# gaocegege/kubeflow-controller

Measured on AMD Instinct MI355X. Metric: images/sec (whole node) ResNet-50 TFJob at 1/2/4/8 workers on MI355X, higher is better.
Workload: dtype bf16; 1 GPU; model=ResNet-50 v1.5, global_batch=256, image=224, per_gpu_batch=256, parallelism=single, optimizer=SGD momentum 0.9 (fused HIP), fp32 master, hip_graph=False

## Files before the change

### csrc/kernels/batchnorm.hip

```cpp
#include <cstdlib>

#include "common.h"

namespace {

constexpr int NT = 256;
constexpr int kSlots = 64;

struct Geom {
  int tpr;
  int rpi;
  int gx;
  long chunk;
};

Geom geom(long M, int C, int max_blocks) {
  Geom g;
  int cv = C / 8;
  g.tpr = cv < NT ? cv : NT;
  g.rpi = NT / g.tpr;
  long want = (M + (long)g.rpi * 8 - 1) / ((long)g.rpi * 8);
  long gx = want < max_blocks ? want : max_blocks;
  if (gx < 1) gx = 1;
  long chunk = (M + gx - 1) / gx;
// ... 266 lines not shown
  {
    const Geom ga = apply_geom(M, C);
    grid = dim3(ga.gx);
    chunk = ga.chunk;
    tpr = ga.tpr;
    rpi = ga.rpi;
  }
  if (rss && relu && res && mb)
    hipLaunchKernelGGL((bn_apply<true, true, true, true>), grid, dim3(NT), 0, s, x, res, y, mb, scale, shift, M, C,
                       chunk, tpr, rpi, rss);
  else if (rss && relu && res)
    hipLaunchKernelGGL((bn_apply<true, true, false, true>), grid, dim3(NT), 0, s, x, res, y, mb, scale, shift, M, C,
                       chunk, tpr, rpi, rss);
  else if (rss && res)
    hipLaunchKernelGGL((bn_apply<false, true, false, true>), grid, dim3(NT), 0, s, x, res, y, mb, scale, shift, M, C,
                       chunk, tpr, rpi, rss);
  else if (relu && res && mb)
    hipLaunchKernelGGL((bn_apply<true, true, true>), grid, dim3(NT), 0, s, x, res, y, mb, scale, shift, M, C, chunk,
                       tpr, rpi);
  else if (relu && res)
    hipLaunchKernelGGL((bn_apply<true, true, false>), grid, dim3(NT), 0, s, x, res, y, mb, scale, shift, M, C, chunk,
                       tpr, rpi);
  else if (relu)
    hipLaunchKernelGGL((bn_apply<true, false, false>), grid, dim3(NT), 0, s, x, res, y, mb, scale, shift, M, C, chunk,
                       tpr, rpi);
  else if (res)
    hipLaunchKernelGGL((bn_apply<false, true, false>), grid, dim3(NT), 0, s, x, res, y, mb, scale, shift, M, C, chunk,
                       tpr, rpi);
  else
    hipLaunchKernelGGL((bn_apply<false, false, false>), grid, dim3(NT), 0, s, x, res, y, mb, scale, shift, M, C,
                       chunk, tpr, rpi);
}

template <int MASK>
__device__ __forceinline__ void masked_dy(const uint4 dv, const uint4 yv, const float xf[8], const float sc[8],
                                          const float sf[8], unsigned bits, float dz[8]) {
  unpack8(dv, dz);
  if (MASK == 3) {
#pragma unroll
    for (int j = 0; j < 8; j++) dz[j] = ((bits >> j) & 1u) ? dz[j] : 0.f;
  } else if (MASK == 1) {
    float yy[8];
    unpack8(yv, yy);
#pragma unroll
    for (int j = 0; j < 8; j++) dz[j] = yy[j] > 0.f ? dz[j] : 0.f;
  } else if (MASK == 2) {
#pragma unroll
    for (int j = 0; j < 8; j++) dz[j] = fmaf(xf[j], sc[j], sf[j]) > 0.f ? dz[j] : 0.f;
  }
}

template <int MASK>
__device__ __forceinline__ void load_ss(const float* __restrict__ ss, int C, int c0, float sc[8], float sf[8]) {
#pragma unroll
  for (int j = 0; j < 8; j++) {
    sc[j] = MASK == 2 ? ss[c0 + j] : 0.f;
    sf[j] = MASK == 2 ? ss[C + c0 + j] : 0.f;
  }
}

template <int MASK>
__global__ __launch_bounds__(NT) void bn_bwd_partial(const bf16_t* __restrict__ dy, const bf16_t* __restrict__ x,
                                                     const bf16_t* __restrict__ y, const uint8_t* __restrict__ mb,
                                                     const float* __restrict__ ss,
                                                     const float* __restrict__ mean, float* __restrict__ part, long M,
                                                     int C, long chunk, int tpr, int rpi) {
  __shared__ __attribute__((aligned(16))) float sh[kRedFloats];
  const int t = threadIdx.x;
  const int cg = t % tpr, r0 = t / tpr;
  const bool active = r0 < rpi;
  const int cv = C / 8;
  const long rb = (long)blockIdx.x * chunk;
  const long re = rb + chunk < M ? rb + chunk : M;
  for (int g0 = 0; g0 < cv; g0 += tpr) {
    const int c0 = (g0 + cg) * 8;
    float s1[8] = {0, 0, 0, 0, 0, 0, 0, 0}, s2[8] = {0, 0, 0, 0, 0, 0, 0, 0};
    if (active && g0 + cg < cv) {
      float mu[8], sc[8], sf[8];
#pragma unroll
      for (int j = 0; j < 8; j++) mu[j] = mean[c0 + j];
      load_ss<MASK>(ss, C, c0, sc, sf);
      long r = rb + r0;
      for (; r + rpi < re; r += 2L * rpi) {
// ... 442 lines not shown
```

### csrc/kernels/common.h

```cpp
#pragma once
#include <hip/hip_runtime.h>
#include <stdint.h>

#define KFA_API extern "C" __attribute__((visibility("default")))

typedef uint16_t bf16_t;
typedef __attribute__((ext_vector_type(8))) short short8;
typedef __attribute__((ext_vector_type(4))) float floatx4;
typedef __attribute__((ext_vector_type(16))) float floatx16;

__device__ __forceinline__ float bf2f(uint32_t b) { return __uint_as_float(b << 16); }

typedef __attribute__((ext_vector_type(2))) __bf16 kfa_bf16x2_t;
typedef __attribute__((ext_vector_type(2))) float kfa_floatx2_t;

__device__ __forceinline__ uint32_t pack2(float lo, float hi) {
  const kfa_floatx2_t f = {lo, hi};
  return __builtin_bit_cast(uint32_t, __builtin_convertvector(f, kfa_bf16x2_t));
}

__device__ __forceinline__ uint32_t f2bf(float f) { return pack2(f, 0.f) & 0xffffu; }

__device__ __forceinline__ void unpack8(const uint4 v, float f[8]) {
  f[0] = __uint_as_float(v.x << 16); f[1] = __uint_as_float(v.x & 0xffff0000u);
  f[2] = __uint_as_float(v.y << 16); f[3] = __uint_as_float(v.y & 0xffff0000u);
  f[4] = __uint_as_float(v.z << 16); f[5] = __uint_as_float(v.z & 0xffff0000u);
  f[6] = __uint_as_float(v.w << 16); f[7] = __uint_as_float(v.w & 0xffff0000u);
}

__device__ __forceinline__ uint4 pack8(const float f[8]) {
  return make_uint4(pack2(f[0], f[1]), pack2(f[2], f[3]), pack2(f[4], f[5]), pack2(f[6], f[7]));
}

__device__ __forceinline__ float wave_sum(float v) {
#pragma unroll
  for (int o = 32; o > 0; o >>= 1) v += __shfl_xor(v, o, 64);
  return v;
}

__device__ __forceinline__ float wave_max(float v) {
#pragma unroll
  for (int o = 32; o > 0; o >>= 1) v = fmaxf(v, __shfl_xor(v, o, 64));
  return v;
}

__device__ __forceinline__ float erf_as(float x, float& e) {
  const float a = fabsf(x);
  const float t = __builtin_amdgcn_rcpf(fmaf(0.3275911f, a, 1.f));
  e = __expf(-a * a);
  const float poly =
      t * fmaf(t, fmaf(t, fmaf(t, fmaf(t, 1.061405429f, -1.453152027f), 1.421413741f), -0.284496736f), 0.254829592f);
  return copysignf(1.f - poly * e, x);
}
__device__ __forceinline__ float gelu_f(float z) {
  float e;
  return 0.5f * z * (1.f + erf_as(z * 0.70710678118654752f, e));
}
__device__ __forceinline__ float gelu_grad(float z) {
  float e;
  const float cdf = 0.5f * (1.f + erf_as(z * 0.70710678118654752f, e));
  return fmaf(z * 0.39894228040143268f, e, cdf);
}

__device__ __forceinline__ uint32_t drop_hash(uint64_t seed, uint64_t i) {
// ... 24 lines not shown
```

### csrc/kernels/pool.hip

```cpp
#include <cstdlib>

#include "common.h"

namespace {

template <typename IT>
__global__ __launch_bounds__(256) void maxpool_fwd(const bf16_t* __restrict__ x, bf16_t* __restrict__ y,
                                                   uint8_t* __restrict__ idx, int N, int H, int W, int C, int Ho,
                                                   int Wo, int k, int s, int p) {
  const IT cv = C / 8;
  const IT total = (IT)N * Ho * Wo * cv;
  for (IT v = (IT)blockIdx.x * blockDim.x + threadIdx.x; v < total; v += (IT)gridDim.x * blockDim.x) {
    const int cg = (int)(v % cv);
    IT t = v / cv;
    const int ow = (int)(t % (IT)Wo);
    t /= (IT)Wo;
    const int oh = (int)(t % (IT)Ho);
    const int n = (int)(t / (IT)Ho);
    float best[8];
    int bi[8];
#pragma unroll
    for (int j = 0; j < 8; j++) { best[j] = -INFINITY; bi[j] = 0; }
    for (int kh = 0; kh < k; kh++) {
      const int ih = oh * s - p + kh;
// ... 212 lines not shown
  for (int a = 0; a < 2; a++)
#pragma unroll
    for (int b = 0; b < 2; b++) {
      const int oh = oh1 - a, ow = ow1 - b;
      const int kh = ih - (oh * 2 - p), kw = iw - (ow * 2 - p);
      const int w = a * 2 + b;
      ok[w] = oh >= 0 && oh < Ho && ow >= 0 && ow < Wo && kh < 3 && kw < 3;
      pos[w] = kh * 3 + kw;
      const long o = (((long)n * Ho + min(max(oh, 0), Ho - 1)) * Wo + min(max(ow, 0), Wo - 1)) * C + cg * 8;
      g[w] = *reinterpret_cast<const uint4*>(dy + o);
      pk[w] = *reinterpret_cast<const uint2*>(idx + o);
    }
  float acc[8] = {0, 0, 0, 0, 0, 0, 0, 0};
#pragma unroll
  for (int w = 0; w < 4; w++) {
    if (!ok[w]) continue;
    float f[8];
    unpack8(g[w], f);
    const uint32_t q[2] = {pk[w].x, pk[w].y};
#pragma unroll
    for (int j = 0; j < 8; j++)
      if ((int)((q[j >> 2] >> ((j & 3) * 8)) & 0xff) == pos[w]) acc[j] += f[j];
  }
  *reinterpret_cast<uint4*>(dx + (long)v * 8) = pack8(acc);
}

struct PoolBnStats {
  const bf16_t* x;
  const float* ss;
  const float* mean;
  float* slots;
};

template <bool STATS>
__global__ __launch_bounds__(256) void maxpool3s2_bwd4(const bf16_t* __restrict__ dy, const uint8_t* __restrict__ idx,
                                                       bf16_t* __restrict__ dx, int N, int H, int W, int C, int Ho,
                                                       int Wo, int p, int T, int U, PoolBnStats bs) {
  const unsigned cv = C / 8;
  const unsigned total = (unsigned)N * T * U * cv;
  const unsigned v = blockIdx.x * blockDim.x + threadIdx.x;
  if (!STATS && v >= total) return;
  const bool live = v < total;
  float s1[8] = {0, 0, 0, 0, 0, 0, 0, 0}, s2[8] = {0, 0, 0, 0, 0, 0, 0, 0};
  float mu[8], sc[8], sf[8];
  const int cg = (int)(v % cv);
  if (STATS)
#pragma unroll
    for (int j = 0; j < 8; j++) {
      mu[j] = bs.mean[cg * 8 + j];
      sc[j] = bs.ss[cg * 8 + j];
      sf[j] = bs.ss[C + cg * 8 + j];
    }
  unsigned q = v / cv;
  const int u = (int)(q % (unsigned)U);
  q /= (unsigned)U;
  const int t = (int)(q % (unsigned)T);
  const int n = live ? (int)(q / (unsigned)T) : 0;
  uint4 g[4];
  uint2 pk[4];
  bool ok[4];
#pragma unroll
  for (int b = 0; b < 2; b++)
#pragma unroll
    for (int e = 0; e < 2; e++) {
      const int oh = t - 1 + b, ow = u - 1 + e, w = b * 2 + e;
      ok[w] = live && oh >= 0 && oh < Ho && ow >= 0 && ow < Wo;
      const long o = (((long)n * Ho + min(max(oh, 0), Ho - 1)) * Wo + min(max(ow, 0), Wo - 1)) * C + cg * 8;
      g[w] = *reinterpret_cast<const uint4*>(dy + o);
      pk[w] = *reinterpret_cast<const uint2*>(idx + o);
    }
#pragma unroll
  for (int a = 0; a < 2; a++)
#pragma unroll
    for (int c = 0; c < 2; c++) {
      const int ih = 2 * t - p + a, iw = 2 * u - p + c;
      if (!live || ih < 0 || ih >= H || iw < 0 || iw >= W) continue;
      float acc[8] = {0, 0, 0, 0, 0, 0, 0, 0};
#pragma unroll
      for (int b = 0; b < 2; b++)
#pragma unroll
        for (int e = 0; e < 2; e++) {
          const int kh = a + 2 - 2 * b, kw = c + 2 - 2 * e;
          const int w = b * 2 + e;
          if (kh > 2 || kw > 2 || !ok[w]) continue;
          const int pos = kh * 3 + kw;
          float f[8];
          unpack8(g[w], f);
          const uint32_t qq[2] = {pk[w].x, pk[w].y};
#pragma unroll
          for (int j = 0; j < 8; j++)
            if ((int)((qq[j >> 2] >> ((j & 3) * 8)) & 0xff) == pos) acc[j] += f[j];
        }
      const long o = (((long)n * H + ih) * W + iw) * C + cg * 8;
      const uint4 packed = pack8(acc);
      *reinterpret_cast<uint4*>(dx + o) = packed;
      if (STATS) {
        float dz[8], xf[8];
        unpack8(packed, dz);
        unpack8(*reinterpret_cast<const uint4*>(bs.x + o), xf);
#pragma unroll
        for (int j = 0; j < 8; j++) {
          const float d = fmaf(xf[j], sc[j], sf[j]) > 0.f ? dz[j] : 0.f;
          s1[j] += d;
          s2[j] += d * (xf[j] - mu[j]);
        }
      }
    }
  if (STATS) {
#pragma unroll
    for (int o = 8; o < 64; o <<= 1)
#pragma unroll
      for (int j = 0; j < 8; j++) { s1[j] += __shfl_xor(s1[j], o, 64); s2[j] += __shfl_xor(s2[j], o, 64); }
    const int lane = threadIdx.x & 63, jj = lane >> 3;
    float a1 = s1[0], a2 = s2[0];
#pragma unroll
    for (int j = 1; j < 8; j++) {
      a1 = jj == j ? s1[j] : a1;
      a2 = jj == j ? s2[j] : a2;
    }
    const int ch = (lane & 7) * 8 + jj;
    float* slot = bs.slots + (long)(blockIdx.x % 64) * 2 * C;
    __hip_atomic_fetch_add(slot + ch, a1, __ATOMIC_RELAXED, __HIP_MEMORY_SCOPE_AGENT);
    __hip_atomic_fetch_add(slot + C + ch, a2, __ATOMIC_RELAXED, __HIP_MEMORY_SCOPE_AGENT);
  }
}

bool pool_bwd4() {
  static int v = -1;
  if (v < 0) {
    const char* e = getenv("KFA_POOL_BWD4");
    v = (e && e[0] == '0') ? 0 : 1;
  }
  return v == 1;
}

int grid_for(long work) {
  long b = (work + 255) / 256;
  return (int)(b < (1L << 20) ? (b < 1 ? 1 : b) : (1L << 20));
}

bool pool_pairs() {
  static int v = -1;
  if (v < 0) {
    const char* e = getenv("KFA_POOL_PAIRS");
    v = (e && e[0] == '0') ? 0 : 1;
  }
  return v == 1;
}

}

KFA_API int kfa_maxpool_fwd(const bf16_t* x, bf16_t* y, uint8_t* idx, int N, int H, int W, int C, int Ho, int Wo,
                            int k, int s, int p, hipStream_t st) {
  if (C % 8 || k > 15) return -1;
  const long work = (long)N * Ho * Wo * (C / 8);
  if (k == 3 && s == 2 && p <= 1 && work < (1L << 31) && (long)N * H * W * C < (1L << 40) && pool_pairs())
    hipLaunchKernelGGL(maxpool3s2_fwd2<false>, dim3((unsigned)(((long)N * Ho * ((Wo + 1) / 2) * (C / 8) + 255) / 256)),
// ... 12 lines not shown

KFA_API int kfa_maxpool_bwd(const bf16_t* dy, const uint8_t* idx, bf16_t* dx, int N, int H, int W, int C, int Ho,
                            int Wo, int k, int s, int p, hipStream_t st) {
  if (C % 8 || k > 15) return -1;
  const long work = (long)N * H * W * (C / 8);
  const int T = (H + p + 1) / 2, U = (W + p + 1) / 2;
  const long work4 = (long)N * T * U * (C / 8);
  if (k == 3 && s == 2 && p <= 1 && pool_bwd4() && work4 < (1L << 31))
    hipLaunchKernelGGL(maxpool3s2_bwd4<false>, dim3((unsigned)((work4 + 255) / 256)), dim3(256), 0, st, dy, idx, dx, N,
                       H, W, C, Ho, Wo, p, T, U, PoolBnStats{nullptr, nullptr, nullptr, nullptr});
  else if (k == 3 && s == 2 && p <= 1 && work < (1L << 31))
    hipLaunchKernelGGL(maxpool3s2_bwd, dim3((unsigned)((work + 255) / 256)), dim3(256), 0, st, dy, idx, dx, N, H, W, C,
                       Ho, Wo, p);
  else if (work < (1L << 31))
    hipLaunchKernelGGL(maxpool_bwd<unsigned>, dim3(grid_for(work)), dim3(256), 0, st, dy, idx, dx, N, H, W, C, Ho, Wo,
                       k, s, p);
  else
    hipLaunchKernelGGL(maxpool_bwd<long>, dim3(grid_for(work)), dim3(256), 0, st, dy, idx, dx, N, H, W, C, Ho, Wo, k,
                       s, p);
  return kfa_status();
}

KFA_API int kfa_maxpool_bwd_bnstats(const bf16_t* dy, const uint8_t* idx, bf16_t* dx, int N, int H, int W, int C,
                                    int Ho, int Wo, int p, const bf16_t* x, const float* ss, const float* mean,
                                    float* slots, hipStream_t st) {
  const int T = (H + p + 1) / 2, U = (W + p + 1) / 2;
  const long work4 = (long)N * T * U * (C / 8);
  if (C != 64 || p > 1 || work4 >= (1L << 31) || !x || !ss || !mean || !slots) return -1;
  hipLaunchKernelGGL(maxpool3s2_bwd4<true>, dim3((unsigned)((work4 + 255) / 256)), dim3(256), 0, st, dy, idx, dx, N, H,
                     W, C, Ho, Wo, p, T, U, PoolBnStats{x, ss, mean, slots});
  return kfa_status();
}

KFA_API int kfa_maxpool_fwd_bn(const bf16_t* x, bf16_t* y, uint8_t* idx, int N, int H, int W, int C, int Ho, int Wo,
                               int k, int s, int p, const float* ss, hipStream_t st) {
  const long work = (long)N * Ho * Wo * (C / 8);
  if (C % 8 || k != 3 || s != 2 || p > 1 || !ss || work >= (1L << 31) || (long)N * H * W * C >= (1L << 40)) return -1;
  if (pool_pairs()) {
    const long w2 = (long)N * Ho * ((Wo + 1) / 2) * (C / 8);
    hipLaunchKernelGGL(maxpool3s2_fwd2<true>, dim3((unsigned)((w2 + 255) / 256)), dim3(256), 0, st, x, y, idx, N, H,
                       W, C, Ho, Wo, p, ss);
  } else {
    hipLaunchKernelGGL(maxpool3s2_fwd<true>, dim3((unsigned)((work + 255) / 256)), dim3(256), 0, st, x, y, idx, N, H,
                       W, C, Ho, Wo, p, ss);
  }
  return kfa_status();
}

namespace {
__global__ __launch_bounds__(256) void gap_fwd_kernel(const bf16_t* __restrict__ x, bf16_t* __restrict__ y, int N, int HW,
                                                      int C) {
  const int cv = C / 8;
  const int t = blockIdx.x * blockDim.x + threadIdx.x;
  if (t >= N * cv) return;
  const int n = t / cv, c8 = t - n * cv;
  const bf16_t* p = x + (long)n * HW * C + c8 * 8;
  float s[8] = {0.f, 0.f, 0.f, 0.f, 0.f, 0.f, 0.f, 0.f};
  int i = 0;
  for (; i + 3 < HW; i += 4) {
    uint4 v[4];
#pragma unroll
    for (int u = 0; u < 4; u++) v[u] = *reinterpret_cast<const uint4*>(p + (long)(i + u) * C);
#pragma unroll
    for (int u = 0; u < 4; u++) {
      float f[8];
      unpack8(v[u], f);
// ... 48 lines not shown
```

### kubeflow_controller_amd/ops/batchnorm.py

```python
from __future__ import annotations

import os

import torch
import torch.nn as nn

from . import _lib
from ..parallel.flat import direct_grad_view, notify_grad_ready


MASK_FROM_X = os.environ.get("KFA_BN_MASK_FROM_X", "1") != "0"


def _as_rows(t: torch.Tensor) -> torch.Tensor:
    if t.dim() == 4:
        if not t.is_contiguous(memory_format=torch.channels_last):
            t = t.contiguous(memory_format=torch.channels_last)
    elif not t.is_contiguous():
        t = t.contiguous()
    return t


def _mc(t: torch.Tensor):
    C = t.shape[1] if t.dim() == 4 else t.shape[-1]
# ... 240 lines not shown
        for p, g, d in ((w, dg, direct), (b, db, direct), (rw, rdg, rdirect), (rb, rdb, rdirect)):
            if d:
                notify_grad_ready(p)
                out.append(None)
            else:
                out.append(g if p.dtype == torch.float32 else g.to(p.dtype))
        return (dx, out[0], out[1], None, None, dr, out[2], out[3], None, None, None, None, None, None, None, None)


def bn_act_dual(bn: "BatchNorm2dAct", x: torch.Tensor, bn_r: "BatchNorm2dAct", r: torch.Tensor,
                bwd_link: bool = False) -> torch.Tensor:
    if not (x.is_cuda and bn.training and bn_r.training and not bn_r.relu and bn.eps == bn_r.eps
            and bn.momentum == bn_r.momentum):
        if getattr(r, "_kfa_prestats_tag", None) == DS_SLOTS:
            bn_slot_workspace(r.shape[1], r.device, DS_SLOTS).zero_()
            r._kfa_prestats = False
        return bn(x, residual=bn_r(r), bwd_link=bwd_link)
    link = BnBwdLink() if bwd_link else None
    rpre = getattr(r, "_kfa_prestats", False) and getattr(r, "_kfa_prestats_tag", None) == DS_SLOTS
    if getattr(r, "_kfa_prestats", False) and not rpre:
        raise ValueError("bn_act_dual: r's statistics must be accumulated into the DS_SLOTS workspace")
    y = _BNDualFn.apply(x, bn.weight, bn.bias, bn.running_mean, bn.running_var, r, bn_r.weight, bn_r.bias,
                        bn_r.running_mean, bn_r.running_var, bn.momentum, bn.eps, bn.relu,
                        getattr(x, "_kfa_prestats", False), rpre, link)
    if link is not None:
        y._kfa_bn_link = link
    return y


_lib.register("kfa_maxpool_fwd_bn", [_lib.P, _lib.P, _lib.P] + [_lib.I] * 9 + [_lib.P, _lib.P])
_lib.register("kfa_maxpool_bwd", [_lib.P, _lib.P, _lib.P] + [_lib.I] * 9 + [_lib.P])
_lib.register("kfa_maxpool_bwd_bnstats", [_lib.P, _lib.P, _lib.P] + [_lib.I] * 7 + [_lib.P] * 5)
POOL_BN_STATS = os.environ.get("KFA_POOL_BN_STATS", "1") != "0"


class _BNReluPoolFn(torch.autograd.Function):

    @staticmethod
    def forward(ctx, x, weight, bias, running_mean, running_var, momentum, eps, prestats, k, s, p):
        x = _as_rows(x)
        N, C, H, W = x.shape
        M = N * H * W
        dev = x.device
        Ho, Wo = (H + 2 * p - k) // s + 1, (W + 2 * p - k) // s + 1
        slots, _ = _workspaces(C, dev)
        f32 = dict(dtype=torch.float32, device=dev)
        mean, invstd, ss = torch.empty(C, **f32), torch.empty(C, **f32), torch.empty(2 * C, **f32)
        st = _lib.stream()
        _lib.call("kfa_bn_finalize", _lib.ptr(x), _lib.ptr(slots), M, C, _lib.ptr(weight), _lib.ptr(bias),
                  _lib.ptr(running_mean), _lib.ptr(running_var), _lib.ptr(mean), _lib.ptr(invstd), _lib.ptr(ss),
                  eps, momentum, int(prestats), st)
        cl = torch.channels_last
        y = torch.empty((N, C, Ho, Wo), dtype=x.dtype, device=dev, memory_format=cl)
        idx = torch.empty((N, C, Ho, Wo), dtype=torch.uint8, device=dev, memory_format=cl)
        _lib.call("kfa_maxpool_fwd_bn", _lib.ptr(x), _lib.ptr(y), _lib.ptr(idx), N, H, W, C, Ho, Wo, k, s, p,
                  _lib.ptr(ss), st)
        ctx.save_for_backward(x, ss, idx, weight, mean, invstd)
        ctx.meta = (N, C, H, W, Ho, Wo, k, s, p)
        ctx.params = (weight, bias)
        return y

    @staticmethod
    def backward(ctx, dy):
        x, ss, idx, weight, mean, invstd = ctx.saved_tensors
        N, C, H, W, Ho, Wo, k, s, p = ctx.meta
        dev = x.device
        st = _lib.stream()
        dy = dy.contiguous(memory_format=torch.channels_last)
        dbn = torch.empty_like(x)
        w, b = ctx.params
        dg, db, direct = _param_grads(w, b, C, dev)
        slots, coef = _workspaces(C, dev)
        dx = torch.empty_like(x)
        if POOL_BN_STATS and C == 64 and k == 3 and s == 2:
            _lib.call("kfa_maxpool_bwd_bnstats", _lib.ptr(dy), _lib.ptr(idx), _lib.ptr(dbn), N, H, W, C, Ho, Wo, p,
                      _lib.ptr(x), _lib.ptr(ss), _lib.ptr(mean), _lib.ptr(slots), st)
            _lib.call("kfa_bn_bwd_prestats", _lib.ptr(dbn), _lib.ptr(x), None, _lib.ptr(weight), _lib.ptr(mean),
                      _lib.ptr(invstd), _lib.ptr(dx), None, _lib.ptr(dg), _lib.ptr(db), _lib.ptr(slots),
                      _lib.ptr(coef), N * H * W, C, 1, int(direct), _lib.ptr(ss), None, st)
        else:
            _lib.call("kfa_maxpool_bwd", _lib.ptr(dy), _lib.ptr(idx), _lib.ptr(dbn), N, H, W, C, Ho, Wo, k, s, p, st)
            _lib.call("kfa_bn_bwd", _lib.ptr(dbn), _lib.ptr(x), None, _lib.ptr(weight), _lib.ptr(mean),
                      _lib.ptr(invstd), _lib.ptr(dx), None, _lib.ptr(dg), _lib.ptr(db), _lib.ptr(slots),
                      _lib.ptr(coef), N * H * W, C, 1, int(direct), _lib.ptr(ss), None, st)
        if direct:
            notify_grad_ready(w)
            notify_grad_ready(b)
            return dx, None, None, None, None, None, None, None, None, None, None
        return (dx, dg if w.dtype == torch.float32 else dg.to(w.dtype), db if b.dtype == torch.float32 else db.to(b.dtype),
                None, None, None, None, None, None, None, None)


def bn_relu_maxpool(bn: "BatchNorm2dAct", x: torch.Tensor, k: int = 3, s: int = 2, p: int = 1) -> torch.Tensor:
    if (x.is_cuda and bn.training and bn.relu and MASK_FROM_X and k == 3 and s == 2 and p <= 1 and x.dim() == 4
            and x.dtype == torch.bfloat16 and x.shape[1] % 8 == 0):
        pre = getattr(x, "_kfa_prestats", False) and getattr(x, "_kfa_prestats_tag", "bn_slots") == "bn_slots"
        return _BNReluPoolFn.apply(x, bn.weight, bn.bias, bn.running_mean, bn.running_var, bn.momentum, bn.eps, pre,
                                   k, s, p)
    from .pool import max_pool2d
    return max_pool2d(bn(x), k, s, p)


def bn_act_reference(x, weight, bias, running_mean, running_var, residual=None, training=True, momentum=0.1,
                     eps=1e-5, relu=True):
    xf = x.float()
    y = torch.nn.functional.batch_norm(xf, running_mean, running_var, weight, bias, training, momentum, eps)
    if residual is not None:
# ... 34 lines not shown
```

### csrc/kernels/conv2_bwd.hip

```cpp
#include "common.h"
#include "tile.h"
#include "conv_epilogue.h"

int kfa_wgrad_reduce_launch(const float* part, int splits, long total, void* grad, int grad_f32, int accumulate,
                            hipStream_t s);

namespace {
using namespace tile;

constexpr int TP2 = 256;
constexpr int HRP2 = 384;
constexpr int NT2 = 512;
constexpr int LR2 = HRP2 * 8 / NT2;

__device__ __forceinline__ int halo_swz2(int row) { return ((row >> 1) & 3) << 1; }

__device__ __forceinline__ unsigned lds_addr2(const void* p) {
  return (unsigned)(uintptr_t)(__attribute__((address_space(3))) const void*)p;
}
template <int OFF>
__device__ __forceinline__ short8 lds_rd16(unsigned la) {
  short8 v;
  asm volatile("ds_read_b128 %0, %1 offset:%2" : "=v"(v) : "v"(la), "i"(OFF) : "memory");
  return v;
}
typedef unsigned uintx4 __attribute__((ext_vector_type(4)));
__device__ __forceinline__ void lds_wr16(unsigned la, uint4 v) {
  const uintx4 w = {v.x, v.y, v.z, v.w};
  asm volatile("ds_write_b128 %0, %1" ::"v"(la), "v"(w) : "memory");
}
__device__ __forceinline__ void lds_wr2(unsigned la, unsigned v) {
  asm volatile("ds_write_b16 %0, %1" ::"v"(la), "v"(v) : "memory");
}
__device__ __forceinline__ short8 and8(const short8 a, const short8 m) {
  const uint4 x = __builtin_bit_cast(uint4, a), y = __builtin_bit_cast(uint4, m);
  return __builtin_bit_cast(short8, make_uint4(x.x & y.x, x.y & y.y, x.z & y.z, x.w & y.w));
}

__global__ __launch_bounds__(NT2, 1) void conv2_bwd_fused_kernel(
    const bf16_t* __restrict__ G, const bf16_t* __restrict__ X2, const float* __restrict__ coef,
    const float* __restrict__ ss2, const bf16_t* __restrict__ Y1, const bf16_t* __restrict__ Wt,
    bf16_t* __restrict__ DX1, float* __restrict__ part, float* __restrict__ stats, BnBwd bnb, Geo g) {
  __shared__ __attribute__((aligned(16))) bf16_t s_halo[HRP2 * 64];
  __shared__ __attribute__((aligned(16))) bf16_t s_w[9 * 64 * 64];
  __shared__ __attribute__((aligned(16))) bf16_t s_y[TP2 * 64];
  __shared__ __attribute__((aligned(16))) uint16_t s_mask[4 * TP2];
// ... 2 lines not shown
  const int tid = threadIdx.x, lane = tid & 63, wave = __builtin_amdgcn_readfirstlane(tid >> 6);
  const int ntiles = (g.M + TP2 - 1) / TP2, nb = gridDim.x, b = blockIdx.x;
  const int base = ntiles / nb, rem = ntiles % nb;
  const int t0 = b * base + (b < rem ? b : rem), nt = base + (b < rem ? 1 : 0);
  if (nt == 0) return;

  const int HW1 = g.W + 1, HR = TP2 + 2 * HW1;
  const int PQ = g.H * g.W;
  const float rPQ = 1.f / (float)PQ, rQ = 1.f / (float)g.W;
  const __amdgpu_buffer_rsrc_t rG = rsrc(G, g.t_bytes), rX = rsrc(X2, g.t_bytes);
  const __amdgpu_buffer_rsrc_t rY = rsrc(Y1, g.d_bytes), rD = rsrc(DX1, g.d_bytes);
  const bool bstat = stats && bnb.x;
  const EpiRes er{rD, rsrc(DX1, 0u), rsrc(bstat ? (const void*)bnb.x : DX1, bstat ? g.d_bytes : 0u), rsrc(DX1, 0u)};

#pragma unroll
  for (int i = 0; i < 9; i++) {
    const int id = i * NT2 + tid, tap = id >> 9, row = (id >> 3) & 63, c = id & 7;
    const uint4 v = *reinterpret_cast<const uint4*>(Wt + row * 576 + tap * 64 + c * 8);
    *reinterpret_cast<uint4*>(s_w + tap * 4096 + swz128(row, c)) = v;
  }
  if (tid < 192) s_tab[tid] = coef[tid];
  else if (tid < 320) s_tab[tid] = ss2[tid - 192];
  __syncthreads();

  const unsigned halo_la = lds_addr2(s_halo), w_la = lds_addr2(s_w), mask_la = lds_addr2(s_mask);
  const unsigned tab_la = lds_addr2(s_tab);
  const int fr = lane & 15, fq = lane >> 4;

  uint4 gv[LR2], xv[LR2];
  auto issue_regs = [&](int t, bool live) __attribute__((always_inline)) {
    int lt = tid;
    asm volatile("" : "+v"(lt));
    const int fc = lt & 7, r0 = lt >> 3;
    const int p0 = t * TP2 - HW1 + r0;
#pragma unroll
    for (int i = 0; i < LR2; i++) {
      const int row = r0 + 64 * i, pix = p0 + 64 * i;
      const bool ok = live && row < HR && (unsigned)pix < (unsigned)g.M;
      const unsigned off = ok ? (unsigned)(pix * 64 + fc * 8) * 2u : kOOB;
      gv[i] = bload16<0>(rG, off);
      xv[i] = bload16<0>(rX, off);
    }
  };
  auto issue_y = [&](int t, bool live) __attribute__((always_inline)) {
    int ly = lane;
    asm volatile("" : "+v"(ly));
#pragma unroll
    for (int i = 0; i < 4; i++) {
      const int row = (wave * 4 + i) * 8 + (ly >> 3);
      const int vo = (row * 64 + (((ly & 7) ^ img_swz<64>(row)) << 3)) * 2;
      buf_dma16(rY, s_y + (wave * 4 + i) * 512, live ? vo : (int)kOOB, live ? t * (TP2 * 128) : 0);
    }
  };

  floatx4 accw[9][2], accd[4][2];
#pragma unroll
  for (int i = 0; i < 4; i++)
#pragma unroll
    for (int j = 0; j < 2; j++) accd[i][j] = floatx4{0.f, 0.f, 0.f, 0.f};
#pragma unroll
  for (int i = 0; i < 9; i++)
#pragma unroll
    for (int j = 0; j < 2; j++) accw[i][j] = floatx4{0.f, 0.f, 0.f, 0.f};

  unsigned amask[2];

  auto wgrad = [&]() __attribute__((always_inline)) {
    int lw = lane;
    asm volatile("" : "+v"(lw));
    const int gq = lw >> 4, li = lw & 15, q4 = li >> 2, p4 = li & 3;
    const int col = (wave >> 1) * 16 + 4 * p4;
    const unsigned mla = mask_la + (unsigned)(gq * 16);
    const int cb0 = (wave & 1) * 32;
    static_for<8>([&](auto kc) __attribute__((always_inline)) {
      constexpr int ks = decltype(kc)::value;
      const short8 y0 = tr_operand_asm<64, ks>(s_y, cb0, lw);
      const short8 y1 = tr_operand_asm<64, ks>(s_y, cb0 + 16, lw);
      const short8 mr0 = lds_rd16<0 * 512 + ks * 64>(mla), mr2 = lds_rd16<1 * 512 + ks * 64>(mla);
      const short8 mc0 = lds_rd16<2 * 512 + ks * 64>(mla), mc2 = lds_rd16<3 * 512 + ks * 64>(mla);
      v4i16 a, c, an, cn;
      auto rd_tap = [&](auto tc, v4i16& ra, v4i16& rc) __attribute__((always_inline)) {
        constexpr int tap = decltype(tc)::value, r = tap / 3, s = tap % 3;
        const int row = HW1 + (1 - r) * g.W + (1 - s) + 8 * gq + q4;
        const unsigned a_la = halo_la + (unsigned)(row * 128 + ((((col >> 3) ^ halo_swz2(row))) << 4) + (col & 7) * 2);
        const unsigned c_la =
// ... 40 lines not shown
      bf[h][0] = lds_rd16<0 * 2048>(bb);
      bf[h][1] = lds_rd16<1 * 2048>(bb);
      bf[h][2] = lds_rd16<2 * 2048>(bb);
      bf[h][3] = lds_rd16<3 * 2048>(bb);
      af[h][0] = lds_rd16<0>(v0 ? aa : zero_la);
      af[h][1] = lds_rd16<0>(v1 ? aa + 2048 : zero_la);
    };
    rd_half(std::integral_constant<int, 0>{}, std::integral_constant<int, 0>{});
    static_for<9>([&](auto tc) __attribute__((always_inline)) {
      constexpr int tap = decltype(tc)::value;
      rd_half(tc, std::integral_constant<int, 1>{});
      lgkm_wait<6>();
      __builtin_amdgcn_sched_barrier(0);
      static_for<8>([&](auto ic) __attribute__((always_inline)) {
        constexpr int ni = decltype(ic)::value >> 1, mi = decltype(ic)::value & 1;
        accd[ni][mi] = __builtin_amdgcn_mfma_f32_16x16x32_bf16(bf[0][ni], af[0][mi], accd[ni][mi], 0, 0, 0);
      });
      __builtin_amdgcn_sched_barrier(0);
      if constexpr (tap < 8) {
        rd_half(std::integral_constant<int, tap + 1>{}, std::integral_constant<int, 0>{});
        lgkm_wait<6>();
      } else {
        lgkm_wait<0>();
      }
      __builtin_amdgcn_sched_barrier(0);
      static_for<8>([&](auto ic) __attribute__((always_inline)) {
        constexpr int ni = decltype(ic)::value >> 1, mi = decltype(ic)::value & 1;
        accd[ni][mi] = __builtin_amdgcn_mfma_f32_16x16x32_bf16(bf[1][ni], af[1][mi], accd[ni][mi], 0, 0, 0);
      });
      __builtin_amdgcn_sched_barrier(0);
    });
  };

  issue_regs(t0, true);
  issue_y(t0, true);
  for (int it = 0; it < nt; it++) {
    const int t = t0 + it, m0 = t * TP2;
    {
      int lt = tid;
      asm volatile("" : "+v"(lt));
      const int fc = lt & 7, r0 = lt >> 3;
      const unsigned ta = tab_la + (unsigned)(fc * 32);
      const short8 t0a = lds_rd16<0>(ta), t0b = lds_rd16<16>(ta);
      const short8 t1a = lds_rd16<256>(ta), t1b = lds_rd16<256 + 16>(ta);
      const short8 t2a = lds_rd16<512>(ta), t2b = lds_rd16<512 + 16>(ta);
      const short8 t3a = lds_rd16<768>(ta), t3b = lds_rd16<768 + 16>(ta);
      const short8 t4a = lds_rd16<1024>(ta), t4b = lds_rd16<1024 + 16>(ta);
      lgkm_wait<0>();
      __builtin_amdgcn_sched_barrier(0);
      const floatx4 ca[2] = {__builtin_bit_cast(floatx4, t0a), __builtin_bit_cast(floatx4, t0b)};
      const floatx4 cb[2] = {__builtin_bit_cast(floatx4, t1a), __builtin_bit_cast(floatx4, t1b)};
      const floatx4 ck[2] = {__builtin_bit_cast(floatx4, t2a), __builtin_bit_cast(floatx4, t2b)};
      const floatx4 sc[2] = {__builtin_bit_cast(floatx4, t3a), __builtin_bit_cast(floatx4, t3b)};
      const floatx4 sf[2] = {__builtin_bit_cast(floatx4, t4a), __builtin_bit_cast(floatx4, t4b)};
#pragma unroll
      for (int i = 0; i < LR2; i++) {
        float gf[8], xf[8], o[8];
        unpack8(gv[i], gf);
        unpack8(xv[i], xf);
#pragma unroll
        for (int j = 0; j < 8; j++) {
          const float dz = fmaf(xf[j], sc[j >> 2][j & 3], sf[j >> 2][j & 3]) > 0.f ? gf[j] : 0.f;
          o[j] = fmaf(ca[j >> 2][j & 3], dz, fmaf(cb[j >> 2][j & 3], xf[j], ck[j >> 2][j & 3]));
        }
        const int row = r0 + 64 * i;
        const uint4 pk = pack8(o);
        const uint4 v = row < HR ? pk : make_uint4(0u, 0u, 0u, 0u);
        lds_wr16(halo_la + (unsigned)(row * 128 + ((fc ^ halo_swz2(row)) << 4)), v);
      }
      if (wave < 4) {
        const int m = m0 + lt;
        const int n = fdiv(m, PQ, rPQ), rm = m - n * PQ;
        const int p = fdiv(rm, g.W, rQ), q = rm - p * g.W;
        const unsigned la = mask_la + (unsigned)(lt * 2);
        lds_wr2(la, p + 1 < g.H ? 0xffffu : 0u);
        lds_wr2(la + 512, p >= 1 ? 0xffffu : 0u);
        lds_wr2(la + 1024, q + 1 < g.W ? 0xffffu : 0u);
        lds_wr2(la + 1536, q >= 1 ? 0xffffu : 0u);
      }
#pragma unroll
      for (int mi = 0; mi < 2; mi++) {
        const int m = m0 + wave * 32 + mi * 16 + (lt & 15);
        const int n = fdiv(m, PQ, rPQ), rm = m - n * PQ;
        const int p = fdiv(rm, g.W, rQ), q = rm - p * g.W;
        unsigned mk = 0;
#pragma unroll
        for (int r = 0; r < 3; r++)
#pragma unroll
          for (int s = 0; s < 3; s++) {
            const bool ok = (unsigned)(p + 1 - r) < (unsigned)g.H && (unsigned)(q + 1 - s) < (unsigned)g.W;
            mk |= ok ? 1u << (r * 3 + s) : 0u;
          }
        amask[mi] = mk;
      }
    }
    vm_wait<0>();
    issue_regs(t + 1, it + 1 < nt);
    lds_barrier();

    wgrad();
    dgrad();

// ... 61 lines not shown
```

Before: 13720 images/sec.

## Recompute maxpool backward in BN apply to avoid materializing stem dbn tensor

```diff
diff --git a/csrc/kernels/batchnorm.hip b/csrc/kernels/batchnorm.hip
--- a/csrc/kernels/batchnorm.hip
+++ b/csrc/kernels/batchnorm.hip
@@ -322,23 +322,6 @@
                        chunk, tpr, rpi);
 }
 
-template <int MASK>
-__device__ __forceinline__ void masked_dy(const uint4 dv, const uint4 yv, const float xf[8], const float sc[8],
-                                          const float sf[8], unsigned bits, float dz[8]) {
-  unpack8(dv, dz);
-  if (MASK == 3) {
-#pragma unroll
-    for (int j = 0; j < 8; j++) dz[j] = ((bits >> j) & 1u) ? dz[j] : 0.f;
-  } else if (MASK == 1) {
-    float yy[8];
-    unpack8(yv, yy);
-#pragma unroll
-    for (int j = 0; j < 8; j++) dz[j] = yy[j] > 0.f ? dz[j] : 0.f;
-  } else if (MASK == 2) {
-#pragma unroll
-    for (int j = 0; j < 8; j++) dz[j] = fmaf(xf[j], sc[j], sf[j]) > 0.f ? dz[j] : 0.f;
-  }
-}
 
 template <int MASK>
 __device__ __forceinline__ void load_ss(const float* __restrict__ ss, int C, int c0, float sc[8], float sf[8]) {
diff --git a/csrc/kernels/common.h b/csrc/kernels/common.h
--- a/csrc/kernels/common.h
+++ b/csrc/kernels/common.h
@@ -30,6 +30,24 @@
 
 __device__ __forceinline__ uint4 pack8(const float f[8]) {
   return make_uint4(pack2(f[0], f[1]), pack2(f[2], f[3]), pack2(f[4], f[5]), pack2(f[6], f[7]));
+}
+
+template <int MASK>
+__device__ __forceinline__ void masked_dy(const uint4 dv, const uint4 yv, const float xf[8], const float sc[8],
+                                          const float sf[8], unsigned bits, float dz[8]) {
+  unpack8(dv, dz);
+  if (MASK == 3) {
+#pragma unroll
+    for (int j = 0; j < 8; j++) dz[j] = ((bits >> j) & 1u) ? dz[j] : 0.f;
+  } else if (MASK == 1) {
+    float yy[8];
+    unpack8(yv, yy);
+#pragma unroll
+    for (int j = 0; j < 8; j++) dz[j] = yy[j] > 0.f ? dz[j] : 0.f;
+  } else if (MASK == 2) {
+#pragma unroll
+    for (int j = 0; j < 8; j++) dz[j] = fmaf(xf[j], sc[j], sf[j]) > 0.f ? dz[j] : 0.f;
+  }
 }
 
 __device__ __forceinline__ float wave_sum(float v) {
diff --git a/csrc/kernels/pool.hip b/csrc/kernels/pool.hip
--- a/csrc/kernels/pool.hip
+++ b/csrc/kernels/pool.hip
@@ -268,7 +268,48 @@
   float* slots;
 };
 
-template <bool STATS>
+struct PoolWin4 {
+  uint4 g[4];
+  uint2 pk[4];
+  bool ok[4];
+};
+
+__device__ __forceinline__ void pool_win4_load(PoolWin4& wn, const bf16_t* __restrict__ dy,
+                                               const uint8_t* __restrict__ idx, int n, int t, int u, int cg, int C,
+                                               int Ho, int Wo, bool live) {
+#pragma unroll
+  for (int b = 0; b < 2; b++)
+#pragma unroll
+    for (int e = 0; e < 2; e++) {
+      const int oh = t - 1 + b, ow = u - 1 + e, w = b * 2 + e;
+      wn.ok[w] = live && oh >= 0 && oh < Ho && ow >= 0 && ow < Wo;
+      const long o = (((long)n * Ho + min(max(oh, 0), Ho - 1)) * Wo + min(max(ow, 0), Wo - 1)) * C + cg * 8;
+      wn.g[w] = *reinterpret_cast<const uint4*>(dy + o);
+      wn.pk[w] = *reinterpret_cast<const uint2*>(idx + o);
+    }
+}
+
+__device__ __forceinline__ void pool_win4_acc(const PoolWin4& wn, int a, int c, float acc[8]) {
+#pragma unroll
+  for (int j = 0; j < 8; j++) acc[j] = 0.f;
+#pragma unroll
+  for (int b = 0; b < 2; b++)
+#pragma unroll
+    for (int e = 0; e < 2; e++) {
+      const int kh = a + 2 - 2 * b, kw = c + 2 - 2 * e;
+      const int w = b * 2 + e;
+      if (kh > 2 || kw > 2) continue;
+      const int pos = kh * 3 + kw;
+      float f[8];
+      unpack8(wn.g[w], f);
+      const uint32_t qq[2] = {wn.pk[w].x, wn.pk[w].y};
+#pragma unroll
+      for (int j = 0; j < 8; j++)
+        if (wn.ok[w] && (int)((qq[j >> 2] >> ((j & 3) * 8)) & 0xff) == pos) acc[j] += f[j];
+    }
+}
+
+template <bool STATS, bool STORE = true>
 __global__ __launch_bounds__(256) void maxpool3s2_bwd4(const bf16_t* __restrict__ dy, const uint8_t* __restrict__ idx,
                                                        bf16_t* __restrict__ dx, int N, int H, int W, int C, int Ho,
                                                        int Wo, int p, int T, int U, PoolBnStats bs) {
@@ -292,51 +333,35 @@
   q /= (unsigned)U;
   const int t = (int)(q % (unsigned)T);
   const int n = live ? (int)(q / (unsigned)T) : 0;
-  uint4 g[4];
-  uint2 pk[4];
-  bool ok[4];
-#pragma unroll
-  for (int b = 0; b < 2; b++)
-#pragma unroll
-    for (int e = 0; e < 2; e++) {
-      const int oh = t - 1 + b, ow = u - 1 + e, w = b * 2 + e;
-      ok[w] = live && oh >= 0 && oh < Ho && ow >= 0 && ow < Wo;
-      const long o = (((long)n * Ho + min(max(oh, 0), Ho - 1)) * Wo + min(max(ow, 0), Wo - 1)) * C + cg * 8;
-      g[w] = *reinterpret_cast<const uint4*>(dy + o);
-      pk[w] = *reinterpret_cast<const uint2*>(idx + o);
-    }
+  PoolWin4 wn;
+  pool_win4_load(wn, dy, idx, n, t, u, cg, C, Ho, Wo, live);
+  uint4 xv[4];
+  if (STATS && !STORE)
+#pragma unroll
+    for (int w = 0; w < 4; w++) {
+      const int ih = min(max(2 * t - p + (w >> 1), 0), H - 1), iw = min(max(2 * u - p + (w & 1), 0), W - 1);
+      xv[w] = *reinterpret_cast<const uint4*>(bs.x + (((long)n * H + ih) * W + iw) * C + cg * 8);
+    }
+  if (STATS && !STORE) __builtin_amdgcn_sched_barrier(0);
 #pragma unroll
   for (int a = 0; a < 2; a++)
 #pragma unroll
     for (int c = 0; c < 2; c++) {
       const int ih = 2 * t - p + a, iw = 2 * u - p + c;
-      if (!live || ih < 0 || ih >= H || iw < 0 || iw >= W) continue;
-      float acc[8] = {0, 0, 0, 0, 0, 0, 0, 0};
-#pragma unroll
-      for (int b = 0; b < 2; b++)
-#pragma unroll
-        for (int e = 0; e < 2; e++) {
-          const int kh = a + 2 - 2 * b, kw = c + 2 - 2 * e;
-          const int w = b * 2 + e;
-          if (kh > 2 || kw > 2 || !ok[w]) continue;
-          const int pos = kh * 3 + kw;
-          float f[8];
-          unpack8(g[w], f);
-          const uint32_t qq[2] = {pk[w].x, pk[w].y};
-#pragma unroll
-          for (int j = 0; j < 8; j++)
-            if ((int)((qq[j >> 2] >> ((j & 3) * 8)) & 0xff) == pos) acc[j] += f[j];
-        }
+      const bool inimg = live && ih >= 0 && ih < H && iw >= 0 && iw < W;
+      if (STORE && !inimg) continue;
+      float acc[8];
+      pool_win4_acc(wn, a, c, acc);
       const long o = (((long)n * H + ih) * W + iw) * C + cg * 8;
       const uint4 packed = pack8(acc);
-      *reinterpret_cast<uint4*>(dx + o) = packed;
+      if (STORE) *reinterpret_cast<uint4*>(dx + o) = packed;
       if (STATS) {
         float dz[8], xf[8];
         unpack8(packed, dz);
-        unpack8(*reinterpret_cast<const uint4*>(bs.x + o), xf);
+        unpack8(STORE ? *reinterpret_cast<const uint4*>(bs.x + o) : xv[a * 2 + c], xf);
 #pragma unroll
         for (int j = 0; j < 8; j++) {
-          const float d = fmaf(xf[j], sc[j], sf[j]) > 0.f ? dz[j] : 0.f;
+          const float d = (inimg && fmaf(xf[j], sc[j], sf[j]) > 0.f) ? dz[j] : 0.f;
           s1[j] += d;
           s2[j] += d * (xf[j] - mu[j]);
         }
@@ -359,6 +384,75 @@
     __hip_atomic_fetch_add(slot + ch, a1, __ATOMIC_RELAXED, __HIP_MEMORY_SCOPE_AGENT);
     __hip_atomic_fetch_add(slot + C + ch, a2, __ATOMIC_RELAXED, __HIP_MEMORY_SCOPE_AGENT);
   }
+}
+
+__device__ __forceinline__ void pool_bwd4_bn_dx(const PoolWin4& wn, const uint4 xv[4], const float cf[5][8],
+                                                uint4 out[4]) {
+#pragma unroll
+  for (int a = 0; a < 2; a++)
+#pragma unroll
+    for (int c = 0; c < 2; c++) {
+      float acc[8], dz[8], xf[8], o[8];
+      pool_win4_acc(wn, a, c, acc);
+      unpack8(xv[a * 2 + c], xf);
+      masked_dy<2>(pack8(acc), make_uint4(0, 0, 0, 0), xf, cf[3], cf[4], 0u, dz);
+#pragma unroll
+      for (int j = 0; j < 8; j++) o[j] = fmaf(cf[0][j], dz[j], fmaf(cf[1][j], xf[j], cf[2][j]));
+      out[a * 2 + c] = pack8(o);
+    }
+}
+
+__global__ __launch_bounds__(256, 4) void maxpool3s2_bwd4_apply(const bf16_t* __restrict__ dy,
+                                                             const uint8_t* __restrict__ idx,
+                                                             const bf16_t* __restrict__ x,
+                                                             const float* __restrict__ ss,
+                                                             const float* __restrict__ coef, bf16_t* __restrict__ dx,
+                                                             int N, int H, int W, int Ho, int Wo, int p, int T,
+                                                             int U) {
+  constexpr int C = 64, cv = C / 8;
+  __shared__ __attribute__((aligned(16))) float sh[5 * C];
+  const int tid = threadIdx.x;
+  const float c0 = tid < 3 * C ? coef[tid] : ss[tid - 3 * C], c1 = ss[C + (tid & 63)];
+  const unsigned total = (unsigned)N * T * U * cv;
+  const unsigned v = blockIdx.x * blockDim.x + threadIdx.x;
+  const bool live = v < total;
+  const int cg = (int)(v % cv);
+  unsigned q = v / cv;
+  const int u = (int)(q % (unsigned)U);
+  q /= (unsigned)U;
+  const int t = (int)(q % (unsigned)T);
+  const int n = live ? (int)(q / (unsigned)T) : 0;
+  PoolWin4 wn;
+  pool_win4_load(wn, dy, idx, n, t, u, cg, C, Ho, Wo, live);
+  uint4 xv[4];
+  long off[4];
+  bool in[4];
+#pragma unroll
+  for (int a = 0; a < 2; a++)
+#pragma unroll
+    for (int c = 0; c < 2; c++) {
+      const int ih = 2 * t - p + a, iw = 2 * u - p + c, w = a * 2 + c;
+      in[w] = live && ih >= 0 && ih < H && iw >= 0 && iw < W;
+      off[w] = (((long)n * H + min(max(ih, 0), H - 1)) * W + min(max(iw, 0), W - 1)) * C + cg * 8;
+      xv[w] = *reinterpret_cast<const uint4*>(x + off[w]);
+    }
+  __builtin_amdgcn_sched_barrier(0);
+  sh[tid] = c0;
+  sh[256 + (tid & 63)] = c1;
+  __syncthreads();
+  float cf[5][8];
+#pragma unroll
+  for (int r = 0; r < 5; r++) {
+    const float4 lo = *reinterpret_cast<const float4*>(sh + r * C + cg * 8);
+    const float4 hi = *reinterpret_cast<const float4*>(sh + r * C + cg * 8 + 4);
+    cf[r][0] = lo.x; cf[r][1] = lo.y; cf[r][2] = lo.z; cf[r][3] = lo.w;
+    cf[r][4] = hi.x; cf[r][5] = hi.y; cf[r][6] = hi.z; cf[r][7] = hi.w;
+  }
+  uint4 out[4];
+  pool_bwd4_bn_dx(wn, xv, cf, out);
+#pragma unroll
+  for (int w = 0; w < 4; w++)
+    if (in[w]) *reinterpret_cast<uint4*>(dx + off[w]) = out[w];
 }
 
 bool pool_bwd4() {
@@ -437,6 +531,28 @@
   return kfa_status();
 }
 
+KFA_API int kfa_maxpool_bwd_bnstats_only(const bf16_t* dy, const uint8_t* idx, int N, int H, int W, int C, int Ho,
+                                         int Wo, int p, const bf16_t* x, const float* ss, const float* mean,
+                                         float* slots, hipStream_t st) {
+  const int T = (H + p + 1) / 2, U = (W + p + 1) / 2;
+  const long work4 = (long)N * T * U * (C / 8);
+  if (C != 64 || p > 1 || work4 >= (1L << 31) || !dy || !idx || !x || !ss || !mean || !slots) return -1;
+  hipLaunchKernelGGL((maxpool3s2_bwd4<true, false>), dim3((unsigned)((work4 + 255) / 256)), dim3(256), 0, st, dy, idx,
+                     nullptr, N, H, W, C, Ho, Wo, p, T, U, PoolBnStats{x, ss, mean, slots});
+  return kfa_status();
+}
+
+KFA_API int kfa_maxpool_bwd_bnapply(const bf16_t* dy, const uint8_t* idx, const bf16_t* x, const float* ss,
+                                    const float* coef, bf16_t* dx, int N, int H, int W, int C, int Ho, int Wo, int p,
+                                    hipStream_t st) {
+  const int T = (H + p + 1) / 2, U = (W + p + 1) / 2;
+  const long work4 = (long)N * T * U * (C / 8);
+  if (C != 64 || p > 1 || work4 >= (1L << 31) || !dy || !idx || !x || !ss || !coef || !dx) return -1;
+  hipLaunchKernelGGL(maxpool3s2_bwd4_apply, dim3((unsigned)((work4 + 255) / 256)), dim3(256), 0, st, dy, idx, x, ss,
+                     coef, dx, N, H, W, Ho, Wo, p, T, U);
+  return kfa_status();
+}
+
 KFA_API int kfa_maxpool_fwd_bn(const bf16_t* x, bf16_t* y, uint8_t* idx, int N, int H, int W, int C, int Ho, int Wo,
                                int k, int s, int p, const float* ss, hipStream_t st) {
   const long work = (long)N * Ho * Wo * (C / 8);
diff --git a/kubeflow_controller_amd/ops/batchnorm.py b/kubeflow_controller_amd/ops/batchnorm.py
--- a/kubeflow_controller_amd/ops/batchnorm.py
+++ b/kubeflow_controller_amd/ops/batchnorm.py
@@ -296,6 +296,9 @@
 _lib.register("kfa_maxpool_bwd", [_lib.P, _lib.P, _lib.P] + [_lib.I] * 9 + [_lib.P])
 _lib.register("kfa_maxpool_bwd_bnstats", [_lib.P, _lib.P, _lib.P] + [_lib.I] * 7 + [_lib.P] * 5)
 POOL_BN_STATS = os.environ.get("KFA_POOL_BN_STATS", "1") != "0"
+_lib.register("kfa_maxpool_bwd_bnstats_only", [_lib.P, _lib.P] + [_lib.I] * 7 + [_lib.P] * 5)
+_lib.register("kfa_maxpool_bwd_bnapply", [_lib.P] * 6 + [_lib.I] * 7 + [_lib.P])
+STEM_BWD_ONEPASS = os.environ.get("KFA_STEM_BWD_ONEPASS", "1") != "0"
 
 
 class _BNReluPoolFn(torch.autograd.Function):
@@ -331,12 +334,21 @@
         dev = x.device
         st = _lib.stream()
         dy = dy.contiguous(memory_format=torch.channels_last)
-        dbn = torch.empty_like(x)
         w, b = ctx.params
         dg, db, direct = _param_grads(w, b, C, dev)
         slots, coef = _workspaces(C, dev)
         dx = torch.empty_like(x)
-        if POOL_BN_STATS and C == 64 and k == 3 and s == 2:
+        fused = POOL_BN_STATS and C == 64 and k == 3 and s == 2
+        dbn = None if (fused and STEM_BWD_ONEPASS) else torch.empty_like(x)
+        if fused and STEM_BWD_ONEPASS:
+            _lib.call("kfa_maxpool_bwd_bnstats_only", _lib.ptr(dy), _lib.ptr(idx), N, H, W, C, Ho, Wo, p,
+                      _lib.ptr(x), _lib.ptr(ss), _lib.ptr(mean), _lib.ptr(slots), st)
+            _lib.call("kfa_bn_bwd_finalize_only", None, _lib.ptr(x), None, _lib.ptr(weight), _lib.ptr(mean),
+                      _lib.ptr(invstd), _lib.ptr(dg), _lib.ptr(db), _lib.ptr(slots), _lib.ptr(coef), N * H * W, C,
+                      1, int(direct), _lib.ptr(ss), None, 1, st)
+            _lib.call("kfa_maxpool_bwd_bnapply", _lib.ptr(dy), _lib.ptr(idx), _lib.ptr(x), _lib.ptr(ss),
+                      _lib.ptr(coef), _lib.ptr(dx), N, H, W, C, Ho, Wo, p, st)
+        elif fused:
             _lib.call("kfa_maxpool_bwd_bnstats", _lib.ptr(dy), _lib.ptr(idx), _lib.ptr(dbn), N, H, W, C, Ho, Wo, p,
                       _lib.ptr(x), _lib.ptr(ss), _lib.ptr(mean), _lib.ptr(slots), st)
             _lib.call("kfa_bn_bwd_prestats", _lib.ptr(dbn), _lib.ptr(x), None, _lib.ptr(weight), _lib.ptr(mean),
```

After: 13780 images/sec (median of 6 runs). Within noise of the previous version (+0.4%).

## Reuse halo rows across tiles in conv2 backward instead of recomputing them

Applied to the files above, without the earlier changes.

```diff
diff --git a/csrc/kernels/conv2_bwd.hip b/csrc/kernels/conv2_bwd.hip
--- a/csrc/kernels/conv2_bwd.hip
+++ b/csrc/kernels/conv2_bwd.hip
@@ -11,7 +11,8 @@
 constexpr int TP2 = 256;
 constexpr int HRP2 = 384;
 constexpr int NT2 = 512;
-constexpr int LR2 = HRP2 * 8 / NT2;
+constexpr int LR2 = TP2 * 8 / NT2;
+constexpr int LP2 = 2;
 
 __device__ __forceinline__ int halo_swz2(int row) { return ((row >> 1) & 3) << 1; }
 
@@ -80,11 +81,11 @@
     int lt = tid;
     asm volatile("" : "+v"(lt));
     const int fc = lt & 7, r0 = lt >> 3;
-    const int p0 = t * TP2 - HW1 + r0;
+    const int p0 = t * TP2 + HW1 + r0;
 #pragma unroll
     for (int i = 0; i < LR2; i++) {
-      const int row = r0 + 64 * i, pix = p0 + 64 * i;
-      const bool ok = live && row < HR && (unsigned)pix < (unsigned)g.M;
+      const int pix = p0 + 64 * i;
+      const bool ok = live && pix < g.M;
       const unsigned off = ok ? (unsigned)(pix * 64 + fc * 8) * 2u : kOOB;
       gv[i] = bload16<0>(rG, off);
       xv[i] = bload16<0>(rX, off);
@@ -99,6 +100,36 @@
       const int vo = (row * 64 + (((ly & 7) ^ img_swz<64>(row)) << 3)) * 2;
       buf_dma16(rY, s_y + (wave * 4 + i) * 512, live ? vo : (int)kOOB, live ? t * (TP2 * 128) : 0);
     }
+  };
+
+  struct Tab2 {
+    floatx4 ca[2], cb[2], ck[2], sc[2], sf[2];
+  };
+  auto read_tab = [&](int fc) __attribute__((always_inline)) {
+    const unsigned ta = tab_la + (unsigned)(fc * 32);
+    const short8 t0a = lds_rd16<0>(ta), t0b = lds_rd16<16>(ta);
+    const short8 t1a = lds_rd16<256>(ta), t1b = lds_rd16<256 + 16>(ta);
+    const short8 t2a = lds_rd16<512>(ta), t2b = lds_rd16<512 + 16>(ta);
+    const short8 t3a = lds_rd16<768>(ta), t3b = lds_rd16<768 + 16>(ta);
+    const short8 t4a = lds_rd16<1024>(ta), t4b = lds_rd16<1024 + 16>(ta);
+    lgkm_wait<0>();
+    __builtin_amdgcn_sched_barrier(0);
+    return Tab2{{__builtin_bit_cast(floatx4, t0a), __builtin_bit_cast(floatx4, t0b)},
+                {__builtin_bit_cast(floatx4, t1a), __builtin_bit_cast(floatx4, t1b)},
+                {__builtin_bit_cast(floatx4, t2a), __builtin_bit_cast(floatx4, t2b)},
+                {__builtin_bit_cast(floatx4, t3a), __builtin_bit_cast(floatx4, t3b)},
+                {__builtin_bit_cast(floatx4, t4a), __builtin_bit_cast(floatx4, t4b)}};
+  };
+  auto form = [&](const Tab2& T, const uint4 gq, const uint4 xq) __attribute__((always_inline)) {
+    float gf[8], xf[8], o[8];
+    unpack8(gq, gf);
+    unpack8(xq, xf);
+#pragma unroll
+    for (int j = 0; j < 8; j++) {
+      const float dz = fmaf(xf[j], T.sc[j >> 2][j & 3], T.sf[j >> 2][j & 3]) > 0.f ? gf[j] : 0.f;
+      o[j] = fmaf(T.ca[j >> 2][j & 3], dz, fmaf(T.cb[j >> 2][j & 3], xf[j], T.ck[j >> 2][j & 3]));
+    }
+    return pack8(o);
   };
 
   floatx4 accw[9][2], accd[4][2];
@@ -205,42 +236,46 @@
     });
   };
 
-  issue_regs(t0, true);
-  issue_y(t0, true);
+  {
+    int lt = tid;
+    asm volatile("" : "+v"(lt));
+    const int fc = lt & 7, r0 = lt >> 3;
+    uint4 pg[LP2], px[LP2];
+#pragma unroll
+    for (int j = 0; j < LP2; j++) {
+      const int prow = r0 + 64 * j, pix = t0 * TP2 - HW1 + prow;
+      const bool ok = prow < 2 * HW1 && (unsigned)pix < (unsigned)g.M;
+      const unsigned off = ok ? (unsigned)(pix * 64 + fc * 8) * 2u : kOOB;
+      pg[j] = bload16<0>(rG, off);
+      px[j] = bload16<0>(rX, off);
+    }
+    issue_regs(t0, true);
+    issue_y(t0, true);
+    const Tab2 T = read_tab(fc);
+#pragma unroll
+    for (int j = 0; j < LP2; j++) {
+      const int prow = r0 + 64 * j;
+      const uint4 v = form(T, pg[j], px[j]);
+      if (prow < 2 * HW1) lds_wr16(halo_la + (unsigned)((TP2 + prow) * 128 + ((fc ^ halo_swz2(prow)) << 4)), v);
+    }
+    if (lt < 8) lds_wr16(halo_la + (unsigned)(HR * 128 + lt * 16), make_uint4(0u, 0u, 0u, 0u));
+  }
+  lds_barrier();
+
   for (int it = 0; it < nt; it++) {
     const int t = t0 + it, m0 = t * TP2;
     {
       int lt = tid;
       asm volatile("" : "+v"(lt));
       const int fc = lt & 7, r0 = lt >> 3;
-      const unsigned ta = tab_la + (unsigned)(fc * 32);
-      const short8 t0a = lds_rd16<0>(ta), t0b = lds_rd16<16>(ta);
-      const short8 t1a = lds_rd16<256>(ta), t1b = lds_rd16<256 + 16>(ta);
-      const short8 t2a = lds_rd16<512>(ta), t2b = lds_rd16<512 + 16>(ta);
-      const short8 t3a = lds_rd16<768>(ta), t3b = lds_rd16<768 + 16>(ta);
-      const short8 t4a = lds_rd16<1024>(ta), t4b = lds_rd16<1024 + 16>(ta);
-      lgkm_wait<0>();
-      __builtin_amdgcn_sched_barrier(0);
-      const floatx4 ca[2] = {__builtin_bit_cast(floatx4, t0a), __builtin_bit_cast(floatx4, t0b)};
-      const floatx4 cb[2] = {__builtin_bit_cast(floatx4, t1a), __builtin_bit_cast(floatx4, t1b)};
-      const floatx4 ck[2] = {__builtin_bit_cast(floatx4, t2a), __builtin_bit_cast(floatx4, t2b)};
-      const floatx4 sc[2] = {__builtin_bit_cast(floatx4, t3a), __builtin_bit_cast(floatx4, t3b)};
-      const floatx4 sf[2] = {__builtin_bit_cast(floatx4, t4a), __builtin_bit_cast(floatx4, t4b)};
-#pragma unroll
-      for (int i = 0; i < LR2; i++) {
-        float gf[8], xf[8], o[8];
-        unpack8(gv[i], gf);
-        unpack8(xv[i], xf);
-#pragma unroll
-        for (int j = 0; j < 8; j++) {
-          const float dz = fmaf(xf[j], sc[j >> 2][j & 3], sf[j >> 2][j & 3]) > 0.f ? gf[j] : 0.f;
-          o[j] = fmaf(ca[j >> 2][j & 3], dz, fmaf(cb[j >> 2][j & 3], xf[j], ck[j >> 2][j & 3]));
-        }
-        const int row = r0 + 64 * i;
-        const uint4 pk = pack8(o);
-        const uint4 v = row < HR ? pk : make_uint4(0u, 0u, 0u, 0u);
-        lds_wr16(halo_la + (unsigned)(row * 128 + ((fc ^ halo_swz2(row)) << 4)), v);
-      }
+      const int row0 = 2 * HW1 + r0;
+      const unsigned la0 = halo_la + (unsigned)(row0 * 128 + ((fc ^ halo_swz2(row0)) << 4));
+      const short8 c2 = lds_rd16<2 * 8192>(la0), c3 = lds_rd16<3 * 8192>(la0);
+      const Tab2 T = read_tab(fc);
+      if (row0 + 128 >= TP2) lds_wr16(la0 + 2 * 8192 - TP2 * 128, __builtin_bit_cast(uint4, c2));
+      if (row0 + 192 >= TP2) lds_wr16(la0 + 3 * 8192 - TP2 * 128, __builtin_bit_cast(uint4, c3));
+#pragma unroll
+      for (int i = 0; i < LR2; i++) lds_wr16(la0 + (unsigned)(i * 8192), form(T, gv[i], xv[i]));
       if (wave < 4) {
         const int m = m0 + lt;
         const int n = fdiv(m, PQ, rPQ), rm = m - n * PQ;
```

Measured after the change: 13960 images/sec before, 14000 images/sec after, median of 6. About the same (+0.3%).
